# CIS565-Fall-2014/Project3-Pathtracer

Hardware: NVIDIA B200
Metric: path segments per second, reference sample scene 800x800, 5000 spp, 8 bounces (higher is better)
Workload: dtype f32

## Files before the change

### include/pt_b200.h

```cpp
#ifndef PT_B200_H
#define PT_B200_H

#include <stddef.h>
#include <stdint.h>

#ifdef __cplusplus
extern "C" {
#endif

#define PT_ABI_VERSION 1

typedef enum {
  PT_OK = 0,
  PT_ERR_INVALID = -1,
  PT_ERR_CUDA = -2,
  PT_ERR_IO = -3,
  PT_ERR_PARSE = -4,
  PT_ERR_STATE = -5
} pt_status;


typedef struct {
  int32_t type;
  int32_t materialid;
// ... 61 lines not shown
int pt_resolve_rgba8(pt_context* ctx, uint32_t spp, uint8_t* host_rgba8, void* device_rgba8);
int pt_accum_device_ptr(pt_context* ctx, void** device_ptr, size_t* bytes);

int pt_reduce_to_first(pt_context* const* ctxs, int n);

int pt_counters(pt_context* ctx, uint64_t* paths, uint64_t* segments, uint64_t* live);
int pt_launch_count(pt_context* ctx, uint64_t* launches);

int pt_raygen(pt_context* ctx, uint64_t seed, int n, const uint32_t* pixel, const uint32_t* sample, float* origin,
              float* direction);
int pt_intersect(pt_context* ctx, int n, const float* origin, const float* direction, int32_t* geom_id, float* t,
                 float* point, float* normal);
int pt_compact_u32(int device, const uint32_t* values, const uint8_t* flags, uint64_t n, uint32_t* out,
                   uint64_t* n_out);
int pt_set_compact_mode(int mode);
int pt_compact_u32_timed(int device, const uint32_t* values, const uint8_t* flags, uint64_t n, uint32_t* out,
                         uint64_t* n_out, int iters, float* kernel_ms);

#define PT_HIT_FILTERED 0
#define PT_HIT_EXACT_SCAN 1
int pt_intersect_ex(pt_context* ctx, int mode, int n, const float* origin, const float* direction, int32_t* geom_id,
                    float* t, float* point, float* normal, uint64_t* fallbacks);
int pt_set_filter_scale(pt_context* ctx, float scale);
int pt_filter_stats(pt_context* ctx, uint64_t* fallbacks);
int pt_filter_retries(pt_context* ctx, uint64_t* retries);

int pt_selftest_math(int device, uint64_t bad[3]);

int pt_set_direct_lighting(pt_context* ctx, int on);
int pt_set_subsurface(pt_context* ctx, int on);
int pt_shadow_rays(pt_context* ctx, uint64_t* shadow_rays, int* n_lights);

int pt_random_points_on_geom(int device, const pt_static_geom* geom, int n, const float* seeds, float* points);
int pt_points_on_geom_u(int device, const pt_static_geom* geom, int n, const float* u, float* points);
int pt_random_directions_in_sphere(int device, int n, const float* xi1, const float* xi2, float* dirs);
int pt_calculate_transmission(int device, int n, const float* absorption, const float* distance, float* out);
int pt_sample_medium(int device, int n, const float* absorption, const float* scatter, const float* distance, const float* u,
                     int32_t* scattered, float* s, float* direction, float* weight);

#define PT_STUB_ORDER_DEVICE 0
#define PT_STUB_ORDER_HOST 1
int pt_reference_stub_image(int device, int width, int height, int iterations, int order, float* rgb);

typedef struct pt_scene pt_scene;
int pt_scene_load(const char* path, int rotat_degrees, pt_scene** out);
int pt_scene_free(pt_scene* s);
// ... 13 lines not shown
```

### project3-pathtracer_b200/__init__.py

```python
import ctypes as C
import os

import numpy as np

from . import build as _build

PKG = os.path.dirname(os.path.abspath(__file__))
LIB_PATH = os.path.join(PKG, "libpt_b200.so")

GEOM_DTYPE = np.dtype([("type", "<i4"), ("materialid", "<i4"), ("translation", "<f4", (3,)), ("rotation", "<f4", (3,)),
                       ("scale", "<f4", (3,)), ("transform", "<f4", (16,)), ("inverseTransform", "<f4", (16,))])
MATERIAL_DTYPE = np.dtype([("color", "<f4", (3,)), ("specularExponent", "<f4"), ("specularColor", "<f4", (3,)),
                           ("hasReflective", "<f4"), ("hasRefractive", "<f4"), ("indexOfRefraction", "<f4"),
                           ("hasScatter", "<f4"), ("absorptionCoefficient", "<f4", (3,)),
                           ("reducedScatterCoefficient", "<f4"), ("emittance", "<f4")])
CAMERA_DTYPE = np.dtype([("resolution", "<f4", (2,)), ("position", "<f4", (3,)), ("view", "<f4", (3,)),
                         ("up", "<f4", (3,)), ("fov", "<f4", (2,))])
LENS_DTYPE = np.dtype([("aperture", "<f4"), ("focal_distance", "<f4")])
assert GEOM_DTYPE.itemsize == 172 and MATERIAL_DTYPE.itemsize == 64 and CAMERA_DTYPE.itemsize == 52

SPHERE, CUBE, MESH = 0, 1, 2
HIT_FILTERED, HIT_EXACT_SCAN = 0, 1


# ... 155 lines not shown

    def launch_count(self):
        n = C.c_uint64()
        _check(lib().pt_launch_count(self._h, C.byref(n)))
        return n.value

    def raygen(self, seed, pixel, sample):
        pixel, sample = _arr(pixel, np.uint32).ravel(), _arr(sample, np.uint32).ravel()
        n = pixel.shape[0]
        o, d = np.zeros((n, 3), np.float32), np.zeros((n, 3), np.float32)
        _check(lib().pt_raygen(self._h, C.c_uint64(seed), C.c_int(n), _p(pixel), _p(sample), _p(o), _p(d)))
        return o, d

    def intersect(self, origin, direction, mode=HIT_FILTERED, with_stats=False):
        o, d = _arr(origin, np.float32).reshape(-1, 3), _arr(direction, np.float32).reshape(-1, 3)
        n = o.shape[0]
        gid, t = np.zeros(n, np.int32), np.zeros(n, np.float32)
        p, nr = np.zeros((n, 3), np.float32), np.zeros((n, 3), np.float32)
        fb = C.c_uint64()
        _check(lib().pt_intersect_ex(self._h, C.c_int(mode), C.c_int(n), _p(o), _p(d), _p(gid), _p(t), _p(p), _p(nr),
                                     C.byref(fb)))
        return (gid, t, p, nr, fb.value) if with_stats else (gid, t, p, nr)

    def set_filter_scale(self, scale):
        _check(lib().pt_set_filter_scale(self._h, C.c_float(scale)))

    def filter_retries(self):
        n = C.c_uint64()
        _check(lib().pt_filter_retries(self._h, C.byref(n)))
        return n.value

    def filter_stats(self):
        n = C.c_uint64()
        _check(lib().pt_filter_stats(self._h, C.byref(n)))
        return n.value


def reduce_to_first(contexts):
    arr = (C.c_void_p * len(contexts))(*[c._h for c in contexts])
    _check(lib().pt_reduce_to_first(arr, C.c_int(len(contexts))))


def selftest_math(device=0):
    bad = (C.c_uint64 * 3)()
    _check(lib().pt_selftest_math(C.c_int(device), bad))
    return tuple(int(x) for x in bad)
# ... 130 lines not shown
```

### project3-pathtracer_b200/csrc/pt_api.cu

```cuda
#include "../../include/pt_b200.h"
#include "pt_kernels.cuh"

#include <nvtx3/nvToolsExt.h>

#include <cmath>
#include <cstdarg>
#include <cstdio>
#include <cstring>
#include <string>
#include <algorithm>
#include <atomic>
#include <thread>
#include <functional>
#include <vector>

using namespace ptd;

struct NvtxRange {
  explicit NvtxRange(const char* name) { nvtxRangePushA(name); }
  ~NvtxRange() { nvtxRangePop(); }
};

static thread_local std::string g_err;
extern "C" void pt_set_error_(const char* fmt, ...) {
  char buf[1024];
  va_list ap;
  va_start(ap, fmt);
  vsnprintf(buf, sizeof(buf), fmt, ap);
  va_end(ap);
  g_err = buf;
}
extern "C" const char* pt_last_error(void) { return g_err.c_str(); }
extern "C" int pt_abi_version(void) { return PT_ABI_VERSION; }

#define CU(call)                                                                             \
  do {                                                                                       \
    cudaError_t e_ = (call);                                                                 \
    if (e_ != cudaSuccess) {                                                                 \
      pt_set_error_("%s failed: %s (%s:%d)", #call, cudaGetErrorString(e_), __FILE__, __LINE__); \
      return PT_ERR_CUDA;                                                                    \
    }                                                                                        \
  } while (0)

extern "C" int pt_device_count(int* count) {
  if (!count) { pt_set_error_("count is NULL"); return PT_ERR_INVALID; }
  *count = 0;
  CU(cudaGetDeviceCount(count));
  return PT_OK;
}

struct pt_context {
  int device = 0;
  int sm_count = 0;
  cudaStream_t own_stream = nullptr, stream = nullptr;
  cudaEvent_t ev0 = nullptr, ev1 = nullptr;
  bool timed = false;
  int n_geoms = 0, n_mats = 0;
  float4* d_rows = nullptr;
  int2* d_meta = nullptr;
  float4* d_normals = nullptr;
  float4* d_mats = nullptr;
  float4* d_lights = nullptr;
  float* d_light_k = nullptr;
  int n_lights = 0;
  bool nee = false;
  bool sss = false;
  int n_media = 0;
  float4* d_filt = nullptr;
  int2* d_filt_ids = nullptr;
  FiltSoA filt{};
  int filt_cap = 0;
  float4* d_bvh_nodes = nullptr;
  float4* d_bvh_leaves = nullptr;
  int2* d_bvh_meta = nullptr;
  BvhSoA bvh{};
  float filter_scale = 1.0f;
  std::vector<pt_static_geom> h_geoms;
  GeomSoA g{};
  RaygenConsts cam{};
  uint32_t W = 0, H = 0, npix = 0;
  uint64_t wf_capacity = 0;
  uint32_t band_pixels = 0;
#ifndef PT_WF_SLOTS
#define PT_WF_SLOTS 2
#endif
  static const int kSlots = PT_WF_SLOTS;
  float4* d_shadow = nullptr;
  uint64_t shadow_cap = 0;
  int shadow_slots = 0;
  int grid_blocks_shadow = 0;
  int shadow_cfg_mode = -1;
  size_t shadow_cfg_smem = 0;
  float4* d_state = nullptr;
  WfCtrl* d_ctrl = nullptr;
  int n_slots = kSlots;
  cudaStream_t wf_stream[kSlots] = {};
  cudaEvent_t ev_fork = nullptr, ev_join[kSlots] = {};
  unsigned long long* d_live = nullptr;
  uint64_t paths_total = 0;
  uint64_t launches = 0;
// ... 53 lines not shown
  *emin = fmin(S[0][0], fmin(S[1][1], S[2][2]));
  *emax = fmax(S[0][0], fmax(S[1][1], S[2][2]));
}
static float round_down(double x) {
  float f = (float)x;
  if ((double)f > x) f = nextafterf(f, -INFINITY);
  return nextafterf(f, -INFINITY);
}
static float round_up(double x) {
  float f = (float)x;
  if ((double)f < x) f = nextafterf(f, INFINITY);
  return nextafterf(f, INFINITY);
}

struct HostFilter {
  std::vector<float4> rows;
  std::vector<int2> ids;
  int end[kFiltClasses] = {0, 0, 0, 0};
  float r_scene = 0.0f;
  std::vector<float4> nodes, leaves;
  std::vector<int2> leaf_meta;
  int root = 0;
  float ew_c_max = 0.0f, ew_w_max = 0.0f;
};
static const int kBvhMinGeoms = 33;
static bool inv3(const double a[3][3], double r[3][3]) {
  const double c00 = a[1][1] * a[2][2] - a[1][2] * a[2][1], c01 = a[1][2] * a[2][0] - a[1][0] * a[2][2],
               c02 = a[1][0] * a[2][1] - a[1][1] * a[2][0];
  const double det = a[0][0] * c00 + a[0][1] * c01 + a[0][2] * c02;
  if (!(fabs(det) > 0) || !std::isfinite(det)) return false;
  const double id = 1.0 / det;
  r[0][0] = c00 * id; r[0][1] = (a[0][2] * a[2][1] - a[0][1] * a[2][2]) * id; r[0][2] = (a[0][1] * a[1][2] - a[0][2] * a[1][1]) * id;
  r[1][0] = c01 * id; r[1][1] = (a[0][0] * a[2][2] - a[0][2] * a[2][0]) * id; r[1][2] = (a[0][2] * a[1][0] - a[0][0] * a[1][2]) * id;
  r[2][0] = c02 * id; r[2][1] = (a[0][1] * a[2][0] - a[0][0] * a[2][1]) * id; r[2][2] = (a[0][0] * a[1][1] - a[0][1] * a[1][0]) * id;
  return true;
}
static HostFilter build_filter(const pt_static_geom* geoms, int n_geoms, double scale) {
  HostFilter F;
  const double u = ldexp(1.0, -24);
  const double s3 = 1.7320508075688772;
  struct Per {
    int geom, cls;
    double KA[3], T[3];
    float k[8];
    float c[3];
    float wk[6];
// ... 166 lines not shown
        r[2] = make_float4(x.wk[1], y.wk[1], x.wk[2], y.wk[2]);
        r[3] = make_float4(x.wk[3], y.wk[3], x.wk[4], y.wk[4]);
        r[4] = make_float4(x.wk[5], y.wk[5], x.ew_c, y.ew_c);
        r[5] = make_float4(x.ew_w, y.ew_w, 0, 0);
      } else {
        const float* A = geoms[x.geom].inverseTransform;
        const float* B = geoms[y.geom].inverseTransform;
        for (int t = 0; t < 3; t++) {
          r[2 * t] = make_float4(A[4 * t], B[4 * t], A[4 * t + 1], B[4 * t + 1]);
          r[2 * t + 1] = make_float4(A[4 * t + 2], B[4 * t + 2], A[4 * t + 3], B[4 * t + 3]);
        }
        if (cls == 1) {
          r[6] = make_float4(x.k[0], y.k[0], x.k[1], y.k[1]);
          r[7] = make_float4(x.k[2], y.k[2], x.ew_c, y.ew_c);
          r[8] = make_float4(x.ew_w, y.ew_w, 0, 0);
        } else {
          r[6] = make_float4(x.k[0], y.k[0], x.k[1], y.k[1]);
          r[7] = make_float4(x.k[2], y.k[2], x.k[3], y.k[3]);
          r[8] = make_float4(x.k[4], y.k[4], x.k[5], y.k[5]);
          r[9] = make_float4(x.ew_c, y.ew_c, x.ew_w, y.ew_w);
        }
      }
      F.rows.insert(F.rows.end(), r, r + kFiltRows);
      F.ids.push_back(make_int2(x.geom, y.geom));
    }
    F.end[cls] = (int)F.ids.size();
  }
  if (F.ids.empty()) { F.rows.assign(kFiltRows, make_float4(0, 0, 0, 0)); F.ids.push_back(make_int2(0, 0)); }

  const int n = (int)per.size();
  if (n >= kBvhMinGeoms) {
    F.leaves.assign((size_t)n * kBvhLeafRows, make_float4(0, 0, 0, 0));
    F.leaf_meta.resize(n);
    for (int k = 0; k < n; k++) {
      const Per& x = per[k];
      float4* L = &F.leaves[(size_t)k * kBvhLeafRows];
      const float* A = geoms[x.geom].inverseTransform;
      if (x.cls == 0) {
        L[0] = make_float4(x.c[0], x.c[1], x.c[2], x.wk[0]);
        L[1] = make_float4(x.wk[1], x.wk[2], x.ew_c, x.ew_w);
        L[2] = make_float4(x.wd[0], 0, 0, 0);
      } else if (x.cls == 2) {
        L[0] = make_float4(x.c[0], x.c[1], x.c[2], x.ew_c);
        L[1] = make_float4(x.wk[0], x.wk[1], x.wk[2], x.ew_w);
        L[2] = make_float4(x.wk[3], x.wk[4], x.wk[5], 0);
        L[3] = make_float4(x.wd[0], x.wd[1], x.wd[2], 0);
// ... 329 lines not shown
    T[3 * k].x = (m.color[0] * m.emittance) * kk;
    T[3 * k].y = (m.color[1] * m.emittance) * kk;
    T[3 * k].z = (m.color[2] * m.emittance) * kk;
  }
  return T;
}

static int upload_filter(pt_context* c) {
  const HostFilter F = build_filter(c->h_geoms.data(), (int)c->h_geoms.size(), (double)c->filter_scale);
  if (F.end[3] != c->filt.end[3] || !c->d_filt) {
    if (c->d_filt) CU(cudaFree(c->d_filt));
    if (c->d_filt_ids) CU(cudaFree(c->d_filt_ids));
    c->d_filt = nullptr; c->d_filt_ids = nullptr;
    CU(cudaMalloc(&c->d_filt, F.rows.size() * sizeof(float4)));
    CU(cudaMalloc(&c->d_filt_ids, F.ids.size() * sizeof(int2)));
  }
  CU(cudaMemcpyAsync(c->d_filt, F.rows.data(), F.rows.size() * sizeof(float4), cudaMemcpyHostToDevice, c->stream));
  CU(cudaMemcpyAsync(c->d_filt_ids, F.ids.data(), F.ids.size() * sizeof(int2), cudaMemcpyHostToDevice, c->stream));
  CU(cudaStreamSynchronize(c->stream));
  c->filt.rows = c->d_filt;
  c->filt.ids = c->d_filt_ids;
  for (int k = 0; k < kFiltClasses; k++) c->filt.end[k] = F.end[k];
  c->filt.r_scene = F.r_scene;
  if (c->d_bvh_nodes) CU(cudaFree(c->d_bvh_nodes));
  if (c->d_bvh_leaves) CU(cudaFree(c->d_bvh_leaves));
  if (c->d_bvh_meta) CU(cudaFree(c->d_bvh_meta));
  c->d_bvh_nodes = nullptr; c->d_bvh_leaves = nullptr; c->d_bvh_meta = nullptr;
  c->bvh = BvhSoA{};
  if (!F.leaf_meta.empty()) {
    CU(cudaMalloc(&c->d_bvh_nodes, F.nodes.size() * sizeof(float4)));
    CU(cudaMalloc(&c->d_bvh_leaves, F.leaves.size() * sizeof(float4)));
    CU(cudaMalloc(&c->d_bvh_meta, F.leaf_meta.size() * sizeof(int2)));
    CU(cudaMemcpy(c->d_bvh_nodes, F.nodes.data(), F.nodes.size() * sizeof(float4), cudaMemcpyHostToDevice));
    CU(cudaMemcpy(c->d_bvh_leaves, F.leaves.data(), F.leaves.size() * sizeof(float4), cudaMemcpyHostToDevice));
    CU(cudaMemcpy(c->d_bvh_meta, F.leaf_meta.data(), F.leaf_meta.size() * sizeof(int2), cudaMemcpyHostToDevice));
    c->bvh.nodes = c->d_bvh_nodes; c->bvh.leaves = c->d_bvh_leaves; c->bvh.leaf_meta = c->d_bvh_meta;
    c->bvh.n_leaves = (int)F.leaf_meta.size(); c->bvh.ew_c_max = F.ew_c_max; c->bvh.ew_w_max = F.ew_w_max;
    c->bvh.root = F.root;
  }
  return PT_OK;
}

static int upload_scene(pt_context* c, const pt_static_geom* geoms, int n_geoms, const pt_material* mats, int n_mats,
                        const pt_camera_data* cam, const pt_lens* lens, bool first) {
  if (!geoms || n_geoms <= 0 || !mats || n_mats <= 0 || !cam) {
    pt_set_error_("geoms, materials and camera are required and must be non-empty");
    return PT_ERR_INVALID;
  }
  const int Wi = (int)cam->resolution[0], Hi = (int)cam->resolution[1];
  if (Wi <= 0 || Hi <= 0 || (uint64_t)Wi * (uint64_t)Hi > (1ull << 31)) {
    pt_set_error_("bad resolution %d x %d", Wi, Hi);
    return PT_ERR_INVALID;
  }
  if (!first && ((uint32_t)Wi != c->W || (uint32_t)Hi != c->H)) {
    pt_set_error_("pt_update_scene cannot change the resolution (%ux%u -> %dx%d)", c->W, c->H, Wi, Hi);
    return PT_ERR_INVALID;
  }
  for (int i = 0; i < n_geoms; i++) {
    if (geoms[i].type <= 1 && (geoms[i].materialid < 0 || geoms[i].materialid >= n_mats)) {
      pt_set_error_("object %d references material %d, but there are %d materials", i, geoms[i].materialid, n_mats);
      return PT_ERR_INVALID;
    }
// ... 60 lines not shown
  c->g.meta = c->d_meta;
  k_normal_table<<<(n_geoms + 127) / 128, 128, 0, c->stream>>>(c->g, n_geoms, reinterpret_cast<const float4*>(c->d_mats), c->d_normals);
  CU(cudaGetLastError());
  c->cam = make_raygen(*cam, lens);
  c->W = (uint32_t)Wi; c->H = (uint32_t)Hi; c->npix = c->W * c->H;
  const int cap = c->filt.end[3] < 1 ? 1 : (c->filt.end[3] < kMaxSmemPairs ? c->filt.end[3] : kMaxSmemPairs);
  const int mode = c->bvh.n_leaves > 0 ? 1 : 0;
  if (cap != c->filt_cap || mode != c->mode) {
    c->filt_cap = cap;
    c->geom_smem = filt_smem_bytes(cap);
    c->mode = mode;
    c->smem_bytes = mode == 0 ? c->geom_smem : kBvhSmemBytes;
    int rc;
    if ((rc = setup_variant<true, false>(c, 0))) return rc;
    if ((rc = setup_variant<true, true>(c, 1))) return rc;
    if ((rc = setup_variant<false, false>(c, 2))) return rc;
    if ((rc = setup_variant<false, true>(c, 3))) return rc;
    if (mode == 0) {
      c->q_smem_total = c->geom_smem + q_smem_bytes();
      if ((rc = setup_variant_q<false>(c, 0))) return rc;
      if ((rc = setup_variant_q<true>(c, 1))) return rc;
    }
    CU(cudaFuncSetAttribute(k_intersect_list, cudaFuncAttributeMaxDynamicSharedMemorySize, (int)c->geom_smem));
  }
  return PT_OK;
}

static size_t state_bytes(uint64_t cap) { return (((size_t)cap * (7 * sizeof(float4))) + 255) & ~(size_t)255; }
static int alloc_wavefront(pt_context* c, uint64_t max_paths) {
  uint64_t spp = max_paths / c->npix;
  if (spp < 1) spp = 1;
  const uint64_t cap = spp * c->npix;
  if (cap > 0xFFFFFF00ull) { pt_set_error_("wavefront of %llu paths exceeds 2^32", (unsigned long long)cap); return PT_ERR_INVALID; }
  if (cap == c->wf_capacity) return PT_OK;
  int n_slots = pt_context::kSlots;
  if (const char* env = getenv("PT_B200_SLOTS")) n_slots = atoi(env) >= 2 ? pt_context::kSlots : 1;
  if (n_slots > 1 && !c->wf_stream[0]) {
    CU(cudaEventCreateWithFlags(&c->ev_fork, cudaEventDisableTiming));
    for (int i = 0; i < pt_context::kSlots; i++) {
      CU(cudaStreamCreateWithFlags(&c->wf_stream[i], cudaStreamNonBlocking));
      CU(cudaEventCreateWithFlags(&c->ev_join[i], cudaEventDisableTiming));
    }
  }
  const uint64_t old_cap = c->wf_capacity;
  const int old_slots = c->n_slots;
  if (c->d_state) CU(cudaFree(c->d_state));
  c->d_state = nullptr; c->wf_capacity = 0;
  if (cudaMalloc(&c->d_state, (size_t)n_slots * state_bytes(cap)) != cudaSuccess) {
// ... 7 lines not shown
    }
    pt_set_error_("cudaMalloc of %llu wavefront paths failed: %s", (unsigned long long)cap, cudaGetErrorString(e));
    return PT_ERR_CUDA;
  }
  c->n_slots = n_slots;
  c->wf_capacity = cap;
  return PT_OK;
}

extern "C" int pt_context_destroy(pt_context* c) {
  if (!c) return PT_OK;
  cudaSetDevice(c->device);
  cudaStream_t streams[] = {c->stream, c->ahead_stream, c->copy_stream, c->wf_stream[0], c->wf_stream[1], c->own_stream};
  for (cudaStream_t st : streams)
    if (st) cudaStreamSynchronize(st);
  const bool dbg = getenv("PT_B200_DEBUG_DESTROY") != nullptr;
  auto chk = [&](cudaError_t e, const char* what) {
    if (e != cudaSuccess && dbg) fprintf(stderr, "pt_context_destroy: %s -> %s\n", what, cudaGetErrorString(e));
  };
#define PT_FREE(p) chk(cudaFree(p), #p)
  PT_FREE(c->d_rows); PT_FREE(c->d_meta); PT_FREE(c->d_normals); PT_FREE(c->d_mats); PT_FREE(c->d_lights); PT_FREE(c->d_state);
  PT_FREE(c->d_filt); PT_FREE(c->d_filt_ids); PT_FREE(c->d_bvh_nodes); PT_FREE(c->d_bvh_leaves); PT_FREE(c->d_bvh_meta);
  PT_FREE(c->d_ctrl); PT_FREE(c->d_live); PT_FREE(c->d_accum); PT_FREE(c->d_rgb); PT_FREE(c->d_rgba8);
  PT_FREE(c->d_scratch); PT_FREE(c->d_light_k); PT_FREE(c->d_shadow);
  PT_FREE(c->d_slab); PT_FREE(c->d_means); PT_FREE(c->d_base[0]); PT_FREE(c->d_base[1]);
#undef PT_FREE
  for (int i = 0; i < pt_context::kSlots; i++) {
    if (c->wf_stream[i]) chk(cudaStreamDestroy(c->wf_stream[i]), "wf_stream");
    if (c->ev_join[i]) chk(cudaEventDestroy(c->ev_join[i]), "ev_join");
  }
  if (c->ev_fork) chk(cudaEventDestroy(c->ev_fork), "ev_fork");
  if (c->ahead_stream) chk(cudaStreamDestroy(c->ahead_stream), "ahead_stream");
  if (c->copy_stream) chk(cudaStreamDestroy(c->copy_stream), "copy_stream");
  if (c->ev_res) chk(cudaEventDestroy(c->ev_res), "ev_res");
  if (c->ev_copy) chk(cudaEventDestroy(c->ev_copy), "ev_copy");
  for (int i = 0; i < 2; i++) {
    if (c->ev_ready[i]) chk(cudaEventDestroy(c->ev_ready[i]), "ev_ready");
    if (c->ev_consumed[i]) chk(cudaEventDestroy(c->ev_consumed[i]), "ev_consumed");
  }
  if (c->h_policy) chk(cudaFreeHost(c->h_policy), "h_policy");
  if (c->ev0) chk(cudaEventDestroy(c->ev0), "ev0");
  if (c->ev1) chk(cudaEventDestroy(c->ev1), "ev1");
  if (c->own_stream) chk(cudaStreamDestroy(c->own_stream), "own_stream");
  cudaGetLastError();
  delete c;
  return PT_OK;
}
// ... 224 lines not shown
      const int in = depth & 1, outb = in ^ 1;
      P.in_o = S + (3 * in + 0) * cap; P.in_d = S + (3 * in + 1) * cap; P.in_t = S + (3 * in + 2) * cap;
      P.out_o = S + (3 * outb + 0) * cap; P.out_d = S + (3 * outb + 1) * cap; P.out_t = S + (3 * outb + 2) * cap;
      P.accum = accum; P.acc_s0 = acc_s0; P.acc_stride = acc_stride;
      P.g = c->g; P.n_geoms = c->n_geoms;
      P.normals = c->d_normals;
      P.filt = c->filt; P.filt_cap = c->filt_cap;
      P.bvh = c->bvh;
      P.bvh_res = S + 6 * cap;
      float4* const SQ = nee_on ? c->d_shadow + (size_t)sl * 4 * cap : nullptr;
      P.sq_o = SQ; P.sq_d = SQ ? SQ + cap : nullptr; P.sq_t = SQ ? SQ + 2 * cap : nullptr; P.sq_x = SQ ? SQ + 3 * cap : nullptr;
      P.mats = c->d_mats;
      P.lights = c->d_lights; P.n_lights = c->n_lights; P.light_k = c->d_light_k;
      P.cam = c->cam;
      P.ctrl = ctrl;
      P.depth = (uint32_t)depth;
      P.keys = philox_keys(seed);
      P.first_sample = first_sample + s0;
      P.n_first = n_first;
      P.pix0 = pix0; P.band = band;
      P.div_band = make_fastdiv(band);
      P.q_offset = (uint32_t)c->geom_smem;
      P.cap = (uint32_t)cap;
      const bool first = depth == 0, last = depth == max_depth - 1;
      cudaError_t e;
      if (first && last) e = launch_bounce<true, true>(c, 1, P, n_first, st);
      else if (first) e = launch_bounce<true, false>(c, 0, P, n_first, st);
      else if (last) e = launch_bounce<false, true>(c, 3, P, n_first, st);
      else e = launch_bounce<false, false>(c, 2, P, n_first, st);
      if (e != cudaSuccess) { pt_set_error_("k_bounce launch failed: %s", cudaGetErrorString(e)); return PT_ERR_CUDA; }
      if (nee_on && !last && (e = launch_shadow(c, P, n_first, st)) != cudaSuccess) {
        pt_set_error_("k_shadow launch failed: %s", cudaGetErrorString(e));
        return PT_ERR_CUDA;
      }
    }
    k_accum_counts<<<1, kMaxDepth, 0, st>>>(ctrl, c->d_live, max_depth, c->q_mode == 0 && !c->mode ? c->d_policy : nullptr);
    c->launches++;
    CU(cudaGetLastError());
    c->paths_total += n_first;
  }
  }
  for (int i = 0; forked && i < slots_used; i++) {
    CU(cudaEventRecord(c->ev_join[i], c->wf_stream[i]));
    CU(cudaStreamWaitEvent(stream0, c->ev_join[i], 0));
  }
  if (timed) {
// ... 260 lines not shown
  CU(cudaMemcpyAsync(dor, origin, v * sizeof(float), cudaMemcpyHostToDevice, c->stream));
  CU(cudaMemcpyAsync(ddr, direction, v * sizeof(float), cudaMemcpyHostToDevice, c->stream));
  CU(cudaMemsetAsync(dfb, 0, sizeof(unsigned long long), c->stream));
  k_intersect_list<<<(n + kTile - 1) / kTile, kTile, c->geom_smem, c->stream>>>(
      c->g, c->n_geoms, c->filt, c->filt_cap, c->bvh, mode == PT_HIT_FILTERED ? c->d_normals : nullptr, mode, n, dor, ddr,
      did, dt, dpnt, dn, dfb);
  c->launches++;
  CU(cudaGetLastError());
  unsigned long long fb = 0;
  CU(cudaMemcpyAsync(geom_id, did, n * sizeof(int), cudaMemcpyDeviceToHost, c->stream));
  CU(cudaMemcpyAsync(t, dt, n * sizeof(float), cudaMemcpyDeviceToHost, c->stream));
  CU(cudaMemcpyAsync(point, dpnt, v * sizeof(float), cudaMemcpyDeviceToHost, c->stream));
  CU(cudaMemcpyAsync(normal, dn, v * sizeof(float), cudaMemcpyDeviceToHost, c->stream));
  CU(cudaMemcpyAsync(&fb, dfb, sizeof(fb), cudaMemcpyDeviceToHost, c->stream));
  CU(cudaStreamSynchronize(c->stream));
  if (fallbacks) *fallbacks = fb;
  return PT_OK;
}
extern "C" int pt_intersect(pt_context* c, int n, const float* origin, const float* direction, int32_t* geom_id,
                            float* t, float* point, float* normal) {
  return pt_intersect_ex(c, PT_HIT_FILTERED, n, origin, direction, geom_id, t, point, normal, nullptr);
}

extern "C" int pt_set_filter_scale(pt_context* c, float scale) {
  CTX(c);
  if (!(scale >= 0.0f) || !(scale <= 1e6f)) { pt_set_error_("filter scale %g outside [0, 1e6]", (double)scale); return PT_ERR_INVALID; }
  CU(cudaStreamSynchronize(c->stream));
  c->filter_scale = scale;
  return upload_filter(c);
}

extern "C" int pt_filter_stats(pt_context* c, uint64_t* fallbacks) {
  CTX(c);
  if (!fallbacks) { pt_set_error_("fallbacks is NULL"); return PT_ERR_INVALID; }
  unsigned long long h = 0;
  CU(cudaMemcpyAsync(&h, c->d_live + kMaxDepth, sizeof(h), cudaMemcpyDeviceToHost, c->stream));
  CU(cudaStreamSynchronize(c->stream));
  *fallbacks = h;
  return PT_OK;
}

extern "C" int pt_filter_retries(pt_context* c, uint64_t* retries) {
  CTX(c);
  if (!retries) { pt_set_error_("retries is NULL"); return PT_ERR_INVALID; }
  unsigned long long h = 0;
  CU(cudaMemcpyAsync(&h, c->d_live + kMaxDepth + 2, sizeof(h), cudaMemcpyDeviceToHost, c->stream));
  CU(cudaStreamSynchronize(c->stream));
  *retries = h;
  return PT_OK;
}

extern "C" int pt_set_direct_lighting(pt_context* c, int on) {
// ... 308 lines not shown
```

### project3-pathtracer_b200/csrc/pt_kernels.cuh

```cuda
#pragma once
#include "pt_device.cuh"
#include "pt_filter.cuh"
#include "pt_bvh.cuh"
#include "pt_sampling.cuh"

namespace ptd {

constexpr int kMaxDepth = 64;
constexpr int kTile = 256;
#ifndef PT_BOUNCE_THREADS
#define PT_BOUNCE_THREADS 256
#endif
constexpr int kBounceThreads = PT_BOUNCE_THREADS;
#ifndef PT_MIN_BLOCKS
#define PT_MIN_BLOCKS 4
#endif

struct WfCtrl {
  uint32_t count[kMaxDepth + 1];
  uint32_t tile_ctr[kMaxDepth + 1];
  uint32_t fallbacks;
  uint32_t retries;
  unsigned long long shadow;
  uint32_t shadow_ctr[kMaxDepth + 1];
// ... 47 lines not shown
  float4* accum;
  GeomSoA g;
  const float4* normals;
  int n_geoms;
  FiltSoA filt;
  int filt_cap;
  BvhSoA bvh;
  float4* bvh_res;
  const float4* mats;
  const float4* lights;
  const float* light_k;
  int n_lights;
  RaygenConsts cam;
  WfCtrl* ctrl;
  uint32_t depth;
  PhiloxKeys keys;
  uint32_t first_sample, n_first;
  uint32_t pix0, band;
  FastDiv div_band;
  float4 *sq_o, *sq_d, *sq_t, *sq_x;
  uint32_t q_offset;
  uint32_t cap;
  uint32_t acc_s0, acc_stride;
};

struct DepthIO {
  const float4 *in_o, *in_d, *in_t;
  float4 *out_o, *out_d, *out_t;
  uint32_t depth;
};
__device__ __forceinline__ DepthIO depth_io(const BounceParams& P) {
  DepthIO io;
  io.in_o = P.in_o; io.in_d = P.in_d; io.in_t = P.in_t;
  io.out_o = P.out_o; io.out_d = P.out_d; io.out_t = P.out_t;
  io.depth = P.depth;
  return io;
}

constexpr int kUnit = 32;

__device__ __forceinline__ void accum_add(float4* px, f3 L) {
  asm volatile("red.global.add.v4.f32 [%0], {%1, %2, %3, %4};" ::"l"(px), "f"(L.x), "f"(L.y), "f"(L.z), "f"(0.0f) : "memory");
}

__device__ __forceinline__ float4* accum_at(const BounceParams& P, uint32_t pixel, uint32_t sample) {
  return P.accum + pixel + (size_t)(sample - P.acc_s0) * P.acc_stride;
}
// ... 212 lines not shown
    const uint32_t idx = unit * kUnit + lane;
    const bool valid = idx < n_in;

    f3 o = mk(0, 0, 0), d = mk(0, 0, 1), thr = mk(1, 1, 1);
    uint32_t pixel = 0, sample = 0;
    float cos_b = 0.0f;
    if (valid) {
      if (FIRST) {
        const uint32_t si = fastdiv(idx, P.div_band);
        pixel = P.pix0 + (idx - si * P.band);
        sample = P.first_sample + si;
        raygen(P.cam, P.keys, pixel, sample, o, d);
      } else {
        const float4 a = __ldcs(io.in_o + idx), b = __ldcs(io.in_d + idx), c = __ldcs(io.in_t + idx);
        o = mk(a.x, a.y, a.z); pixel = __float_as_uint(a.w);
        d = mk(b.x, b.y, b.z); sample = __float_as_uint(b.w);
        thr = mk(c.x, c.y, c.z);
        if (NEE) cos_b = c.w;
      }
    }

    Hit h;
    h.t = INFINITY; h.id = -1; h.p = mk(0, 0, 0); h.ncode = 0;
    if (valid) {
      ScanBest best;
      scan_init(best);
      const ScanRay ray = make_scan_ray(o, d, P.filt.r_scene, P.filt.end[2] > P.filt.end[1]);
      filter_scan(fs, 0, P.filt.end[3], P.filt.end, ray, best);
      if (resolve_scan(best, P.filt, P.g, P.n_geoms, o, d, h)) atomicAdd(&P.ctrl->fallbacks, 1u);
    }

    shade_and_compact<LAST, true, NEE, false, true, MEDIUM>(P, io, fs, lane, valid && h.id >= 0, h, o, d, thr, pixel, sample, cos_b);
    }
  }
}

template <bool FIRST, bool LAST, bool NEE = false, bool MEDIUM = false>
__global__ void __launch_bounds__(kBounceThreads, PT_MIN_BLOCKS) k_bounce(const __grid_constant__ BounceParams P) {
  extern __shared__ __align__(16) unsigned char smem_raw[];
  stage_filt(P.filt, 0, P.filt.end[3], reinterpret_cast<float4*>(smem_raw));
  __syncthreads();
  bounce_fused<FIRST, LAST, NEE, MEDIUM>(P, depth_io(P), reinterpret_cast<const float4*>(smem_raw), threadIdx.x & 31u);
}

constexpr int kQCap = 96;
#ifndef PT_Q_PREFETCH
#define PT_Q_PREFETCH 1
// ... 561 lines not shown
      scan_init(best);
      bvh_traverse<false>(bvh, g, ray, best, h);
      if (resolve_bvh(best, bvh, g, filt.r_scene, oo, dd, h)) atomicAdd(fallbacks, 1ull);
    }
  } else {
    const float4* fs = reinterpret_cast<const float4*>(smem_raw);
    const ScanRay ray = make_scan_ray(oo, dd, filt.r_scene, filt.end[2] > filt.end[1]);
    ScanBest best;
    scan_init(best);
    stage_filt(filt, 0, filt.end[3], reinterpret_cast<float4*>(smem_raw));
    __syncthreads();
    if (valid) filter_scan(fs, 0, filt.end[3], filt.end, ray, best);
    if (valid && resolve_scan(best, filt, g, n_geoms, oo, dd, h)) atomicAdd(fallbacks, 1ull);
  }
  if (!valid) return;
  f3 nn = mk(0, 0, 0);
  if (h.id >= 0) nn = normals ? hit_normal_table(normals, h) : hit_normal(__ldg(g.fwd0 + h.id), __ldg(g.fwd1 + h.id), __ldg(g.fwd2 + h.id), h);
  id[i] = h.id;
  t[i] = h.id >= 0 ? h.t : -1.0f;
  p[3 * i] = h.p.x; p[3 * i + 1] = h.p.y; p[3 * i + 2] = h.p.z;
  nrm[3 * i] = nn.x; nrm[3 * i + 1] = nn.y; nrm[3 * i + 2] = nn.z;
}

#ifndef PT_COMPACT_THREADS
#define PT_COMPACT_THREADS 256
#endif
constexpr int kCompactThreads = PT_COMPACT_THREADS;
constexpr int kCompactItems = 16;
constexpr int kCompactTile = kCompactThreads * kCompactItems;
#ifndef PT_COMPACT_BLOCKS
#define PT_COMPACT_BLOCKS (2048 / PT_COMPACT_THREADS)
#endif
__global__ void __launch_bounds__(kCompactThreads, PT_COMPACT_BLOCKS) k_compact_u32(const uint32_t* __restrict__ values, const uint8_t* __restrict__ flags,
                                                       uint32_t n, uint32_t* __restrict__ out, uint32_t* n_out,
                                                       uint32_t* ticket, uint64_t* status, uint32_t epoch) {
  __shared__ uint32_t s_tile;
  __shared__ uint32_t s_warp[kCompactThreads / 32];
  __shared__ uint32_t s_base;
  const uint32_t lane = threadIdx.x & 31u, warp = threadIdx.x >> 5;
  const uint32_t lt = (1u << lane) - 1u;
  const uint32_t n_tiles = (n + kCompactTile - 1) / kCompactTile;
  const bool aligned = (reinterpret_cast<uintptr_t>(values) & 15u) == 0 && (reinterpret_cast<uintptr_t>(flags) & 3u) == 0;
  for (;;) {
    __syncthreads();
    if (threadIdx.x == 0) s_tile = atomicAdd(ticket, 1u);
    __syncthreads();
// ... 270 lines not shown
```

Baseline: 29010.

## Precompute per-pixel primary-hit candidate table to skip first-bounce filter scan

For pinhole cameras in pair-scan mode, a per-pixel table is built at scene upload. Each entry bounds the pixel's ray footprint cone and records the nearest candidate geometry together with a conservative bound on the second-nearest entry distance. On the first bounce, rays look up this table and run one exact intersection instead of the full filter scan, falling back to a warp-wide rescan when the candidate check fails. This trades per-frame scan work for a host/device precompute and extra double-precision bookkeeping, with some risk of warp divergence from retries.

```diff
diff --git a/include/pt_b200.h b/include/pt_b200.h
--- a/include/pt_b200.h
+++ b/include/pt_b200.h
@@ -107,6 +107,9 @@
 int pt_intersect_ex(pt_context* ctx, int mode, int n, const float* origin, const float* direction, int32_t* geom_id,
                     float* t, float* point, float* normal, uint64_t* fallbacks);
 int pt_set_filter_scale(pt_context* ctx, float scale);
+int pt_primary_hit(pt_context* ctx, uint64_t seed, int n, const uint32_t* pixel, const uint32_t* sample, int32_t* geom_id,
+                   float* t, float* point, float* normal, uint8_t* decided, uint64_t* fallbacks);
+int pt_primary_table_info(pt_context* ctx, int* active, float* build_ms);
 int pt_filter_stats(pt_context* ctx, uint64_t* fallbacks);
 int pt_filter_retries(pt_context* ctx, uint64_t* retries);
 
diff --git a/project3-pathtracer_b200/__init__.py b/project3-pathtracer_b200/__init__.py
--- a/project3-pathtracer_b200/__init__.py
+++ b/project3-pathtracer_b200/__init__.py
@@ -201,6 +201,23 @@
                                      C.byref(fb)))
         return (gid, t, p, nr, fb.value) if with_stats else (gid, t, p, nr)
 
+    def primary_hit(self, seed, pixel, sample, with_stats=False):
+        pixel, sample = _arr(pixel, np.uint32).ravel(), _arr(sample, np.uint32).ravel()
+        n = pixel.shape[0]
+        gid, t = np.zeros(n, np.int32), np.zeros(n, np.float32)
+        p, nr = np.zeros((n, 3), np.float32), np.zeros((n, 3), np.float32)
+        dec = np.zeros(n, np.uint8)
+        fb = C.c_uint64()
+        _check(lib().pt_primary_hit(self._h, C.c_uint64(seed), C.c_int(n), _p(pixel), _p(sample), _p(gid), _p(t), _p(p),
+                                    _p(nr), _p(dec), C.byref(fb)))
+        out = (gid, t, p, nr, dec.astype(bool))
+        return out + (fb.value,) if with_stats else out
+
+    def primary_table_info(self, time_build=False):
+        on, ms = C.c_int(), C.c_float()
+        _check(lib().pt_primary_table_info(self._h, C.byref(on), C.byref(ms) if time_build else None))
+        return bool(on.value), (ms.value if time_build else None)
+
     def set_filter_scale(self, scale):
         _check(lib().pt_set_filter_scale(self._h, C.c_float(scale)))
 
diff --git a/project3-pathtracer_b200/csrc/pt_api.cu b/project3-pathtracer_b200/csrc/pt_api.cu
--- a/project3-pathtracer_b200/csrc/pt_api.cu
+++ b/project3-pathtracer_b200/csrc/pt_api.cu
@@ -10,6 +10,7 @@
 #include <string>
 #include <algorithm>
 #include <atomic>
+#include <chrono>
 #include <thread>
 #include <functional>
 #include <vector>
@@ -49,6 +50,10 @@
   return PT_OK;
 }
 
+struct FiltGeom {
+  int key, cls, geom;
+  float c[3], k[6], wk[6], ew_c, ew_w;
+};
 struct pt_context {
   int device = 0;
   int sm_count = 0;
@@ -76,6 +81,10 @@
   BvhSoA bvh{};
   float filter_scale = 1.0f;
   std::vector<pt_static_geom> h_geoms;
+  std::vector<FiltGeom> filt_geoms;
+  uint32_t* d_ptab = nullptr;
+  PrimRec* d_prim = nullptr;
+  bool ptab_on = false;
   GeomSoA g{};
   RaygenConsts cam{};
   uint32_t W = 0, H = 0, npix = 0;
@@ -175,6 +184,7 @@
   std::vector<int2> leaf_meta;
   int root = 0;
   float ew_c_max = 0.0f, ew_w_max = 0.0f;
+  std::vector<FiltGeom> geoms;
 };
 static const int kBvhMinGeoms = 33;
 static bool inv3(const double a[3][3], double r[3][3]) {
@@ -387,6 +397,14 @@
         }
       }
       F.rows.insert(F.rows.end(), r, r + kFiltRows);
+      for (int half = 0; half < (dummy ? 1 : 2); half++) {
+        const Per& z = half ? y : x;
+        FiltGeom e;
+        e.key = 2 * (int)F.ids.size() + half; e.cls = cls; e.geom = z.geom;
+        memcpy(e.c, z.c, sizeof(e.c)); memcpy(e.k, z.k, sizeof(e.k)); memcpy(e.wk, z.wk, sizeof(e.wk));
+        e.ew_c = z.ew_c; e.ew_w = z.ew_w;
+        F.geoms.push_back(e);
+      }
       F.ids.push_back(make_int2(x.geom, y.geom));
     }
     F.end[cls] = (int)F.ids.size();
@@ -762,6 +780,7 @@
   c->filt.ids = c->d_filt_ids;
   for (int k = 0; k < kFiltClasses; k++) c->filt.end[k] = F.end[k];
   c->filt.r_scene = F.r_scene;
+  c->filt_geoms = F.geoms;
   if (c->d_bvh_nodes) CU(cudaFree(c->d_bvh_nodes));
   if (c->d_bvh_leaves) CU(cudaFree(c->d_bvh_leaves));
   if (c->d_bvh_meta) CU(cudaFree(c->d_bvh_meta));
@@ -778,6 +797,81 @@
     c->bvh.n_leaves = (int)F.leaf_meta.size(); c->bvh.ew_c_max = F.ew_c_max; c->bvh.ew_w_max = F.ew_w_max;
     c->bvh.root = F.root;
   }
+  return PT_OK;
+}
+
+static int build_primary_table(pt_context* c) {
+  c->ptab_on = false;
+  if (c->mode != 0 || c->cam.aperture > 0.0f || c->filt_geoms.empty() || c->filt_geoms.size() > (size_t)kMaxPrimRecs) return PT_OK;
+  const double up = 1.0 + 1e-6;
+  const double o[3] = {c->cam.eye.x, c->cam.eye.y, c->cam.eye.z};
+  const double omax = fmax(fmax(fabs(o[0]), fabs(o[1])), fabs(o[2]));
+  const double w = (4.0 * omax + (double)c->filt.r_scene) * up;
+  std::vector<PrimRec> recs;
+  for (const FiltGeom& e : c->filt_geoms) {
+    if (e.key >= (int)kKeyMask) return PT_OK;
+    PrimRec r;
+    memset(&r, 0, sizeof(r));
+    r.ball = e.cls <= 1;
+    r.key = e.key;
+    double ctr[3], half[3];
+    if (e.cls == 0 || e.cls == 2) {
+      double oc2 = 0.0;
+      for (int i = 0; i < 3; i++) {
+        r.A[4 * i] = 1.0;
+        ctr[i] = e.c[i];
+        r.ro[i] = o[i] - ctr[i];
+        r.g[i] = 1.0;
+        oc2 += r.ro[i] * r.ro[i];
+      }
+      if (e.cls == 0) {
+        r.h[0] = sqrt(((double)e.wk[0] + (double)e.wk[1] * w + (double)e.wk[2] * oc2) * up);
+        for (int i = 0; i < 3; i++) half[i] = r.h[0];
+      } else {
+        for (int i = 0; i < 3; i++) half[i] = r.h[i] = ((double)e.wk[i] + (double)e.wk[3 + i] * w) * up;
+      }
+    } else {
+      const float* A = c->h_geoms[e.geom].inverseTransform;
+      double A3[3][3], Ai[3][3], AtA[3][3], ro2 = 0.0;
+      for (int i = 0; i < 3; i++) {
+        for (int j = 0; j < 3; j++) { A3[i][j] = A[4 * i + j]; r.A[3 * i + j] = A3[i][j]; }
+        r.ro[i] = (double)A[4 * i] * o[0] + (double)A[4 * i + 1] * o[1] + (double)A[4 * i + 2] * o[2] + (double)A[4 * i + 3];
+        ro2 += r.ro[i] * r.ro[i];
+      }
+      if (!inv3(A3, Ai)) return PT_OK;
+      for (int i = 0; i < 3; i++) ctr[i] = -(Ai[i][0] * A[3] + Ai[i][1] * A[7] + Ai[i][2] * A[11]);
+      if (e.cls == 1) {
+        for (int a = 0; a < 3; a++)
+          for (int b = 0; b < 3; b++) { AtA[a][b] = 0.0; for (int k = 0; k < 3; k++) AtA[a][b] += A3[k][a] * A3[k][b]; }
+        double lmin, lmax;
+        sym3_eigen_range(AtA, &lmin, &lmax);
+        r.h[0] = sqrt(((double)e.k[0] + (double)e.k[1] * w + (double)e.k[2] * ro2) * up);
+        r.g[0] = sqrt(fmax(lmax, 0.0)) * 1.001;
+        for (int i = 0; i < 3; i++) half[i] = r.h[0] * sqrt(Ai[i][0] * Ai[i][0] + Ai[i][1] * Ai[i][1] + Ai[i][2] * Ai[i][2]) * 1.001;
+      } else {
+        for (int i = 0; i < 3; i++) {
+          r.h[i] = ((double)e.k[i] + (double)e.k[3 + i] * w) * up;
+          r.g[i] = sqrt(A3[i][0] * A3[i][0] + A3[i][1] * A3[i][1] + A3[i][2] * A3[i][2]) * 1.001;
+        }
+        for (int i = 0; i < 3; i++) half[i] = (fabs(Ai[i][0]) * r.h[0] + fabs(Ai[i][1]) * r.h[1] + fabs(Ai[i][2]) * r.h[2]) * 1.001;
+      }
+    }
+    double D2 = 0.0;
+    for (int i = 0; i < 3; i++) { const double q = fabs(o[i] - ctr[i]) + half[i]; D2 += q * q; }
+    r.D = sqrt(D2) * 1.001;
+    r.ew = ((double)e.ew_c + (double)e.ew_w * w) * up;
+    bool finite = std::isfinite(r.D) && std::isfinite(r.ew);
+    for (int i = 0; i < 3; i++) finite = finite && std::isfinite(r.ro[i]) && std::isfinite(r.h[i]) && std::isfinite(r.g[i]);
+    if (!finite) return PT_OK;
+    recs.push_back(r);
+  }
+  if (!c->d_ptab) CU(cudaMalloc(&c->d_ptab, (size_t)c->npix * sizeof(uint32_t)));
+  if (!c->d_prim) CU(cudaMalloc(&c->d_prim, (size_t)kMaxPrimRecs * sizeof(PrimRec)));
+  CU(cudaMemcpyAsync(c->d_prim, recs.data(), recs.size() * sizeof(PrimRec), cudaMemcpyHostToDevice, c->stream));
+  k_primary_table<<<(c->npix + 127) / 128, 128, 0, c->stream>>>(c->cam, c->d_prim, (int)recs.size(), (double)c->filter_scale, c->d_ptab);
+  CU(cudaGetLastError());
+  CU(cudaStreamSynchronize(c->stream));
+  c->ptab_on = true;
   return PT_OK;
 }
 
@@ -884,8 +978,9 @@
       if ((rc = setup_variant_q<true>(c, 1))) return rc;
     }
     CU(cudaFuncSetAttribute(k_intersect_list, cudaFuncAttributeMaxDynamicSharedMemorySize, (int)c->geom_smem));
-  }
-  return PT_OK;
+    CU(cudaFuncSetAttribute(k_primary_list, cudaFuncAttributeMaxDynamicSharedMemorySize, (int)c->geom_smem));
+  }
+  return build_primary_table(c);
 }
 
 static size_t state_bytes(uint64_t cap) { return (((size_t)cap * (7 * sizeof(float4))) + 255) & ~(size_t)255; }
@@ -939,7 +1034,7 @@
   PT_FREE(c->d_rows); PT_FREE(c->d_meta); PT_FREE(c->d_normals); PT_FREE(c->d_mats); PT_FREE(c->d_lights); PT_FREE(c->d_state);
   PT_FREE(c->d_filt); PT_FREE(c->d_filt_ids); PT_FREE(c->d_bvh_nodes); PT_FREE(c->d_bvh_leaves); PT_FREE(c->d_bvh_meta);
   PT_FREE(c->d_ctrl); PT_FREE(c->d_live); PT_FREE(c->d_accum); PT_FREE(c->d_rgb); PT_FREE(c->d_rgba8);
-  PT_FREE(c->d_scratch); PT_FREE(c->d_light_k); PT_FREE(c->d_shadow);
+  PT_FREE(c->d_scratch); PT_FREE(c->d_light_k); PT_FREE(c->d_shadow); PT_FREE(c->d_ptab); PT_FREE(c->d_prim);
   PT_FREE(c->d_slab); PT_FREE(c->d_means); PT_FREE(c->d_base[0]); PT_FREE(c->d_base[1]);
 #undef PT_FREE
   for (int i = 0; i < pt_context::kSlots; i++) {
@@ -1210,6 +1305,7 @@
       P.div_band = make_fastdiv(band);
       P.q_offset = (uint32_t)c->geom_smem;
       P.cap = (uint32_t)cap;
+      P.ptab = c->ptab_on ? c->d_ptab : nullptr;
       const bool first = depth == 0, last = depth == max_depth - 1;
       cudaError_t e;
       if (first && last) e = launch_bounce<true, true>(c, 1, P, n_first, st);
@@ -1516,12 +1612,63 @@
   return pt_intersect_ex(c, PT_HIT_FILTERED, n, origin, direction, geom_id, t, point, normal, nullptr);
 }
 
+extern "C" int pt_primary_hit(pt_context* c, uint64_t seed, int n, const uint32_t* pixel, const uint32_t* sample, int32_t* geom_id,
+                              float* t, float* point, float* normal, uint8_t* decided, uint64_t* fallbacks) {
+  CTX(c);
+  if (n < 0 || (n > 0 && (!pixel || !sample || !geom_id || !t || !point || !normal || !decided))) { pt_set_error_("bad arguments"); return PT_ERR_INVALID; }
+  if (c->mode != 0) { pt_set_error_("pt_primary_hit: the scene has %d geoms and uses the hierarchy, not the pair scan", c->n_geoms); return PT_ERR_STATE; }
+  if (fallbacks) *fallbacks = 0;
+  if (n == 0) return PT_OK;
+  for (int i = 0; i < n; i++)
+    if (pixel[i] >= c->npix) { pt_set_error_("pixel[%d] = %u outside the %u-pixel frame", i, pixel[i], c->npix); return PT_ERR_INVALID; }
+  const size_t v = 3 * (size_t)n;
+  Arena A(c);
+  if (int rc = A.reserve(2 * Arena::up(n * sizeof(uint32_t)) + 2 * Arena::up(v * sizeof(float)) + Arena::up(n * sizeof(float)) +
+                         Arena::up(n * sizeof(int)) + Arena::up(n) + 256)) return rc;
+  uint32_t *dp = A.take<uint32_t>(n), *ds = A.take<uint32_t>(n);
+  float *dt = A.take<float>(n), *dpnt = A.take<float>(v), *dn = A.take<float>(v);
+  int* did = A.take<int>(n);
+  uint8_t* ddec = A.take<uint8_t>(n);
+  unsigned long long* dfb = A.take<unsigned long long>(1);
+  CU(cudaMemcpyAsync(dp, pixel, n * sizeof(uint32_t), cudaMemcpyHostToDevice, c->stream));
+  CU(cudaMemcpyAsync(ds, sample, n * sizeof(uint32_t), cudaMemcpyHostToDevice, c->stream));
+  CU(cudaMemsetAsync(dfb, 0, sizeof(unsigned long long), c->stream));
+  k_primary_list<<<(n + kTile - 1) / kTile, kTile, c->geom_smem, c->stream>>>(c->cam, seed, c->g, c->n_geoms, c->filt, c->d_normals,
+                                                                               c->ptab_on ? c->d_ptab : nullptr, n, dp, ds, did, dt, dpnt, dn, ddec, dfb);
+  c->launches++;
+  CU(cudaGetLastError());
+  unsigned long long fb = 0;
+  CU(cudaMemcpyAsync(geom_id, did, n * sizeof(int), cudaMemcpyDeviceToHost, c->stream));
+  CU(cudaMemcpyAsync(t, dt, n * sizeof(float), cudaMemcpyDeviceToHost, c->stream));
+  CU(cudaMemcpyAsync(point, dpnt, v * sizeof(float), cudaMemcpyDeviceToHost, c->stream));
+  CU(cudaMemcpyAsync(normal, dn, v * sizeof(float), cudaMemcpyDeviceToHost, c->stream));
+  CU(cudaMemcpyAsync(decided, ddec, n, cudaMemcpyDeviceToHost, c->stream));
+  CU(cudaMemcpyAsync(&fb, dfb, sizeof(fb), cudaMemcpyDeviceToHost, c->stream));
+  CU(cudaStreamSynchronize(c->stream));
+  if (fallbacks) *fallbacks = fb;
+  return PT_OK;
+}
+
+extern "C" int pt_primary_table_info(pt_context* c, int* active, float* build_ms) {
+  CTX(c);
+  if (!active) { pt_set_error_("active is NULL"); return PT_ERR_INVALID; }
+  *active = c->ptab_on ? 1 : 0;
+  if (build_ms) {
+    CU(cudaStreamSynchronize(c->stream));
+    const auto t0 = std::chrono::steady_clock::now();
+    if (int rc = build_primary_table(c)) return rc;
+    *build_ms = std::chrono::duration<float, std::milli>(std::chrono::steady_clock::now() - t0).count();
+  }
+  return PT_OK;
+}
+
 extern "C" int pt_set_filter_scale(pt_context* c, float scale) {
   CTX(c);
   if (!(scale >= 0.0f) || !(scale <= 1e6f)) { pt_set_error_("filter scale %g outside [0, 1e6]", (double)scale); return PT_ERR_INVALID; }
   CU(cudaStreamSynchronize(c->stream));
   c->filter_scale = scale;
-  return upload_filter(c);
+  if (int rc = upload_filter(c)) return rc;
+  return build_primary_table(c);
 }
 
 extern "C" int pt_filter_stats(pt_context* c, uint64_t* fallbacks) {
diff --git a/project3-pathtracer_b200/csrc/pt_kernels.cuh b/project3-pathtracer_b200/csrc/pt_kernels.cuh
--- a/project3-pathtracer_b200/csrc/pt_kernels.cuh
+++ b/project3-pathtracer_b200/csrc/pt_kernels.cuh
@@ -93,7 +93,153 @@
   uint32_t q_offset;
   uint32_t cap;
   uint32_t acc_s0, acc_stride;
+  const uint32_t* ptab;
 };
+
+struct PrimRec {
+  double A[9];
+  double ro[3];
+  double h[3];
+  double g[3];
+  double D;
+  double ew;
+  int ball, key;
+};
+constexpr int kMaxPrimRecs = 128;
+__device__ __forceinline__ double footprint_angle(const RaygenConsts& C, uint32_t pixel, double dc[3]) {
+  const double u = 5.9604644775390625e-8;
+  const uint32_t yi = pixel / C.W;
+  const double x = (double)(pixel - yi * C.W), y = (double)yi, fw = C.fw, fh = C.fh;
+  const double ex = 16.0 * u * (1.0 + 2.0 * (x + 1.0) / fw), ey = 16.0 * u * (1.0 + 2.0 * (y + 1.0) / fh);
+  const double sx0 = 1.0 - 2.0 * (x + 1.0) / fw - ex, sx1 = 1.0 - 2.0 * x / fw + ex;
+  const double sy0 = 1.0 - 2.0 * (y + 1.0) / fh - ey, sy1 = 1.0 - 2.0 * y / fh + ey;
+  const double w[3] = {C.w.x, C.w.y, C.w.z}, H[3] = {C.Hh.x, C.Hh.y, C.Hh.z}, V[3] = {C.Vv.x, C.Vv.y, C.Vv.z};
+  double n[3] = {H[1] * V[2] - H[2] * V[1], H[2] * V[0] - H[0] * V[2], H[0] * V[1] - H[1] * V[0]};
+  const double nn = sqrt(n[0] * n[0] + n[1] * n[1] + n[2] * n[2]);
+  const double vmin = fabs(w[0] * n[0] + w[1] * n[1] + w[2] * n[2]) / nn;
+  const double nw = sqrt(w[0] * w[0] + w[1] * w[1] + w[2] * w[2]), nH = sqrt(H[0] * H[0] + H[1] * H[1] + H[2] * H[2]),
+               nV = sqrt(V[0] * V[0] + V[1] * V[1] + V[2] * V[2]);
+  const double ev = 8.0 * u * (nw + nH * fmax(fabs(sx0), fabs(sx1)) + nV * fmax(fabs(sy0), fabs(sy1)));
+  if (!(nn > 0) || !(vmin > 16.0 * ev)) return -1.0;
+  const double th_r = 2.0 * ev / vmin + 8.0 * u;
+  const double sxc = 0.5 * (sx0 + sx1), syc = 0.5 * (sy0 + sy1);
+  double l = 0.0;
+  for (int i = 0; i < 3; i++) { dc[i] = w[i] + H[i] * sxc + V[i] * syc; l += dc[i] * dc[i]; }
+  l = sqrt(l);
+  for (int i = 0; i < 3; i++) dc[i] /= l;
+  double th = 0.0;
+  for (int k = 0; k < 4; k++) {
+    const double sx = (k & 1) ? sx1 : sx0, sy = (k & 2) ? sy1 : sy0;
+    double v[3];
+    for (int i = 0; i < 3; i++) v[i] = w[i] + H[i] * sx + V[i] * sy;
+    const double cx = v[1] * dc[2] - v[2] * dc[1], cy = v[2] * dc[0] - v[0] * dc[2], cz = v[0] * dc[1] - v[1] * dc[0];
+    th = fmax(th, atan2(sqrt(cx * cx + cy * cy + cz * cz), v[0] * dc[0] + v[1] * dc[1] + v[2] * dc[2]));
+  }
+  th = (th + th_r) * (1.0 + 1e-6) + 1e-12;
+  return th < 1.0 ? th : -1.0;
+}
+__device__ __forceinline__ double prim_entry(const PrimRec& R, const double rw[3], double rho) {
+  if (R.ball) {
+    const double r = R.h[0] + rho * R.g[0];
+    const double ro2 = R.ro[0] * R.ro[0] + R.ro[1] * R.ro[1] + R.ro[2] * R.ro[2];
+    const double a = rw[0] * rw[0] + rw[1] * rw[1] + rw[2] * rw[2];
+    const double b = R.ro[0] * rw[0] + R.ro[1] * rw[1] + R.ro[2] * rw[2];
+    const double c = ro2 - (r * r + 1e-9 * (ro2 + r * r));
+    const double disc = b * b - a * c;
+    if (disc < 0.0) return INFINITY;
+    const double sq = sqrt(disc);
+    if (-b + sq < 0.0) return INFINITY;
+    return fmax((-b - sq) / a, 0.0);
+  }
+  double tn = 0.0, tf = INFINITY;
+  for (int i = 0; i < 3; i++) {
+    const double h = (R.h[i] + rho * R.g[i]) * (1.0 + 1e-9) + 1e-9 * fabs(R.ro[i]);
+    if (rw[i] == 0.0) {
+      if (fabs(R.ro[i]) > h) return INFINITY;
+      continue;
+    }
+    const double t1 = (-h - R.ro[i]) / rw[i], t2 = (h - R.ro[i]) / rw[i];
+    tn = fmax(tn, fmin(t1, t2));
+    tf = fmin(tf, fmax(t1, t2));
+  }
+  return tn <= tf ? tn : INFINITY;
+}
+__global__ void __launch_bounds__(128) k_primary_table(RaygenConsts C, const PrimRec* recs, int n_recs, double scale, uint32_t* tab) {
+  const uint32_t pixel = blockIdx.x * blockDim.x + threadIdx.x;
+  if (pixel >= C.npix) return;
+  double dc[3];
+  const double th = footprint_angle(C, pixel, dc);
+  uint32_t entry = kKeyMask;
+  if (th >= 0.0) {
+    double lo1 = INFINITY, lo2 = INFINITY;
+    int k1 = -1;
+    for (int j = 0; j < n_recs; j++) {
+      const PrimRec& R = recs[j];
+      double rw[3];
+      for (int i = 0; i < 3; i++) rw[i] = R.A[3 * i] * dc[0] + R.A[3 * i + 1] * dc[1] + R.A[3 * i + 2] * dc[2];
+      const double rho = scale * R.D * th * (1.0 + 1e-6);
+      const double s = prim_entry(R, rw, rho);
+      if (!(s < INFINITY)) continue;
+      const double lo = fmax(s - R.ew, 0.0);
+      if (lo < lo1) { lo2 = lo1; lo1 = lo; k1 = R.key; }
+      else lo2 = fmin(lo2, lo);
+    }
+    if (k1 >= 0 && lo2 > lo1) {
+      float f = (float)fmin(lo2, 3.0e38);
+      if ((double)f > lo2) f = nextafterf(f, 0.0f);
+      entry = (__float_as_uint(f) & ~kKeyMask) | (uint32_t)k1;
+    }
+  }
+  tab[pixel] = entry;
+}
+
+__device__ __forceinline__ bool primary_hit(const uint32_t* tab, const float4* fs, const FiltSoA& filt, const GeomSoA& g, int n_geoms,
+                                            bool valid, uint32_t pixel, f3 o, f3 d, Hit& h, bool& decided) {
+  ScanBest best;
+  best.k1 = -1; best.lo2 = 0.0f;
+  bool scan = valid, open = valid, from_tab = false, fell_back = false;
+  decided = false;
+  if (tab != nullptr && valid) {
+    const uint32_t e = __ldg(tab + pixel);
+    if ((e & kKeyMask) != kKeyMask) {
+      best.k1 = (int)(e & kKeyMask); best.lo2 = __uint_as_float(e & ~kKeyMask);
+      scan = false; from_tab = true;
+    }
+  }
+#pragma unroll 1
+  for (;;) {
+    if (__any_sync(0xffffffffu, scan)) {
+      if (scan) {
+        scan_init(best);
+        const ScanRay ray = make_scan_ray(o, d, filt.r_scene, filt.end[2] > filt.end[1]);
+        filter_scan(fs, 0, filt.end[3], filt.end, ray, best);
+      }
+    }
+    bool retry = false;
+    if (open && best.k1 >= 0) {
+      const int gi = __ldg(reinterpret_cast<const int*>(filt.ids) + best.k1);
+      const int type = best.k1 < 2 * filt.end[1] ? 0 : 1;
+      float dist;
+      f3 P;
+      int ncode;
+      DeferredGuard m;
+      const bool hit = exact_hit(type, __ldg(g.inv0 + gi), __ldg(g.inv1 + gi), __ldg(g.inv2 + gi), __ldg(g.fwd0 + gi),
+                                 __ldg(g.fwd1 + gi), __ldg(g.fwd2 + gi), o, d, dist, P, ncode, m);
+      if (!m.bad && hit && dist > 0 && dist < best.lo2) {
+        h.t = dist; h.id = gi; h.p = P; h.ncode = ncode;
+        decided = from_tab;
+      } else if (from_tab) {
+        retry = true;
+      } else {
+        closest_hit_exact(g, n_geoms, o, d, h);
+        fell_back = true;
+      }
+    }
+    if (!__any_sync(0xffffffffu, retry)) break;
+    scan = retry; open = retry; from_tab = false;
+  }
+  return fell_back;
+}
 
 struct DepthIO {
   const float4 *in_o, *in_d, *in_t;
@@ -352,7 +498,11 @@
 
     Hit h;
     h.t = INFINITY; h.id = -1; h.p = mk(0, 0, 0); h.ncode = 0;
-    if (valid) {
+    if constexpr (FIRST) {
+      PT_CHECK(!valid || pixel < P.cam.npix);
+      bool decided;
+      if (primary_hit(P.ptab, fs, P.filt, P.g, P.n_geoms, valid, pixel, o, d, h, decided)) atomicAdd(&P.ctrl->fallbacks, 1u);
+    } else if (valid) {
       ScanBest best;
       scan_init(best);
       const ScanRay ray = make_scan_ray(o, d, P.filt.r_scene, P.filt.end[2] > P.filt.end[1]);
@@ -960,6 +1110,35 @@
   nrm[3 * i] = nn.x; nrm[3 * i + 1] = nn.y; nrm[3 * i + 2] = nn.z;
 }
 
+__global__ void __launch_bounds__(kTile) k_primary_list(RaygenConsts C, uint64_t seed, GeomSoA g, int n_geoms, FiltSoA filt,
+                                                        const float4* normals, const uint32_t* tab, int n, const uint32_t* pixel,
+                                                        const uint32_t* sample, int* id, float* t, float* p, float* nrm,
+                                                        uint8_t* decided, unsigned long long* fallbacks) {
+  extern __shared__ __align__(16) unsigned char smem_raw[];
+  const int i = blockIdx.x * blockDim.x + threadIdx.x;
+  const bool valid = i < n;
+  stage_filt(filt, 0, filt.end[3], reinterpret_cast<float4*>(smem_raw));
+  __syncthreads();
+  f3 oo = mk(0, 0, 0), dd = mk(0, 0, 1);
+  uint32_t px = 0;
+  if (valid) {
+    px = pixel[i];
+    PT_CHECK(px < C.npix);
+    raygen(C, seed, px, sample[i], oo, dd);
+  }
+  Hit h;
+  h.t = INFINITY; h.id = -1; h.p = mk(0, 0, 0); h.ncode = 0;
+  bool dec;
+  if (primary_hit(tab, reinterpret_cast<const float4*>(smem_raw), filt, g, n_geoms, valid, px, oo, dd, h, dec)) atomicAdd(fallbacks, 1ull);
+  if (!valid) return;
+  const f3 nn = h.id >= 0 ? hit_normal_table(normals, h) : mk(0, 0, 0);
+  id[i] = h.id;
+  t[i] = h.id >= 0 ? h.t : -1.0f;
+  p[3 * i] = h.p.x; p[3 * i + 1] = h.p.y; p[3 * i + 2] = h.p.z;
+  nrm[3 * i] = nn.x; nrm[3 * i + 1] = nn.y; nrm[3 * i + 2] = nn.z;
+  decided[i] = dec ? 1 : 0;
+}
+
 #ifndef PT_COMPACT_THREADS
 #define PT_COMPACT_THREADS 256
 #endif
```

After: 30010, median of 6. 1.03x the previous value.
